# 3DAnimals/3DAnimals

Measured on AMD Instinct MI355X. Metric: train images/sec fwd+bwd @256x256 b16, higher is better.
Workload: dtype f32

## Files before the change

3danimals_amd/_lib.py:

```python
from __future__ import annotations

import ctypes
import os
from typing import NamedTuple

import torch

_HERE = os.path.dirname(os.path.abspath(__file__))
LIB_PATH = os.environ.get("A3D_LIB") or os.path.join(_HERE, "lib", "liba3d_hip.so")

_c_int, _c_float, _c_size_t, _p = ctypes.c_int, ctypes.c_float, ctypes.c_size_t, ctypes.c_void_p


class DmtetOrder(ctypes.Structure):
    _fields_ = [("size", ctypes.c_uint32), ("group_slots", ctypes.c_int32), ("vertex_of_rank", _p), ("edges_ranked", _p), ("edge_of_row", _p),
                ("tets_ranked", _p), ("tet_of_row", _p), ("edge_groups", _p), ("tet_groups", _p)]


class RastOpts(ctypes.Structure):
    _fields_ = [("size", ctypes.c_uint32), ("lists_stride", ctypes.c_int32), ("prev_rast", _p), ("cover_scratch", _p), ("aa_screen", _p),
                ("aa_count", _p), ("topo_off", _p), ("topo_adj", _p), ("topo_opp", _p), ("normals_v_a", _p), ("normals_v_b", _p),
                ("normals_off", _p), ("normals_adj", _p), ("normals_acc_a", _p), ("normals_a", _p), ("normals_acc_b", _p), ("normals_b", _p),
                ("normals_B_a", ctypes.c_int32), ("normals_B_b", ctypes.c_int32), ("defer_resolve", ctypes.c_int32), ("reserved", ctypes.c_int32)]

# ... 253 lines not shown
        "a3d_field_head_scratch_bytes": (_c_size_t, [ctypes.c_int64, _c_int]),
        "a3d_field_head_fwd": (_c_int, [_p, _p, _p, _p, _c_int, ctypes.c_int64, _c_int, _p, _p, _p]),
        "a3d_field_head_bwd": (_c_int, [_p, _p, _p, _p, _p, _c_int, ctypes.c_int64, _c_int, _p, _p, _p, _p]),
    }, {}, {"A3D_FIELD_HEAD_WIDTH": FIELD_HEAD_WIDTH, "A3D_FIELD_HEAD_MAX_C": FIELD_HEAD_MAX_C, "A3D_FIELD_HEAD_WG_ROWS": FIELD_HEAD_WG_ROWS,
            "A3D_FIELD_HEAD_ACT_NONE": FIELD_HEAD_ACT_NONE, "A3D_FIELD_HEAD_ACT_SIGMOID": FIELD_HEAD_ACT_SIGMOID}),
    Surface("a3d_eval.h", {
        "a3d_vertex_visibility_fwd": (_c_int, [_p, _p, _c_int, _c_int, _c_int, _c_int, _c_int, _p, _p, _p]),
        "a3d_nearest_visible_vertex_scratch_bytes": (_c_size_t, [_c_int, _c_int]),
        "a3d_nearest_visible_vertex_slab": (_c_int, [_c_int, _c_int]),
        "a3d_nearest_visible_vertex_fwd": (_c_int, [_p, _p, _p, _c_int, _c_int, _c_int, _p, _p, _p]),
    }, {}, {"A3D_NVV_THREADS": NVV_THREADS, "A3D_NVV_MAX_TRIPS": NVV_MAX_TRIPS, "A3D_NVV_KEYPOINT_TILE": NVV_KEYPOINT_TILE}),
)
SIGNATURES = {name: sig for s in SURFACES for name, sig in s.signatures.items()}
assert len(SIGNATURES) == sum(len(s.signatures) for s in SURFACES), "an entry point is registered in two surfaces"

ABI_VERSION = 405
_lib = None


class A3DError(RuntimeError):
    pass


def lib():
    global _lib
    if _lib is None:
        if not os.path.exists(LIB_PATH):
            raise A3DError(
                f"{LIB_PATH} is missing: build it with `python 3danimals_amd/csrc/build.py` "
                "(or __graft_entry__.build()).  There is no CPU fallback for the HIP hot path."
            )
        handle = ctypes.CDLL(LIB_PATH)
        for name, (res, args) in SIGNATURES.items():
            fn = getattr(handle, name)
            fn.restype, fn.argtypes = res, args
        if handle.a3d_version() != ABI_VERSION:
            raise A3DError(f"{LIB_PATH} has ABI version {handle.a3d_version()}, this package binds version {ABI_VERSION}: rebuild it "
                           "with `python 3danimals_amd/csrc/build.py`")
        _lib = handle
    return _lib


class KernelTimer:

    active = None

    def __init__(self):
        self.records = {}
# ... 22 lines not shown
guard_stats = dict(checks=0, buffers_checked=0, allocations=0)


def set_guard(level):
    global GUARD
    import importlib

    prev, GUARD = GUARD, int(level)
    ops = importlib.import_module(__package__ + ".ops")
    ops.torch = GuardedTorch(torch) if GUARD else torch
    if not GUARD:
        _guard_live.clear()
    return prev


def guarded_empty(shape, dtype, device, zero=False, site=""):
    dtype = dtype or torch.get_default_dtype()
    shape = tuple(int(v) for v in shape)
    n = 1
    for v in shape:
        n *= v
    item = torch.empty((), dtype=dtype).element_size()
    nbytes = n * item
    pad = (-nbytes) % 16
    base = torch.empty(GUARD_BYTES + nbytes + pad + GUARD_BYTES, dtype=torch.uint8, device=device)
    base[:GUARD_BYTES] = _GUARD_BYTE
    base[GUARD_BYTES + nbytes:] = _GUARD_BYTE
    t = base[GUARD_BYTES:GUARD_BYTES + nbytes].view(dtype).view(shape)
    if zero:
        t.zero_()
    elif GUARD >= 2 and n:
        if dtype.is_floating_point:
            t.fill_(float("nan"))
# ... 76 lines not shown
            first = int((t != _GUARD_BYTE).nonzero()[0])
            bad.append(f"{what}: bytes AFTER the buffer overwritten ({int((t != _GUARD_BYTE).sum())}, first {first} bytes past its end)")
            t.fill_(_GUARD_BYTE)
        if not head:
            base[:GUARD_BYTES] = _GUARD_BYTE
    raise A3DError(f"A3D_GUARD: buffer overrun detected after {where}: " + "; ".join(bad))


_HELD = []
_SYNC_EVERY_CALL = os.environ.get("A3D_SYNC_CALLS", "0") == "1"
_TRACE_FILE = open(os.environ["A3D_TRACE_CALLS"], "w") if os.environ.get("A3D_TRACE_CALLS") else None


def call(name: str, *args, tag: str = ""):
    timer = KernelTimer.active
    if _TRACE_FILE is not None:
        _TRACE_FILE.write(f"{name}{tag} {args}\n")
        _TRACE_FILE.flush()
    if timer is not None:
        a, b = torch.cuda.Event(enable_timing=True), torch.cuda.Event(enable_timing=True)
        a.record()
    rc = getattr(lib(), name)(*args)
    del _HELD[:]
    if GUARD and rc == 0:
        guard_check(name + tag)
    if _SYNC_EVERY_CALL:
        try:
            torch.cuda.synchronize()
        except Exception as e:
            raise A3DError(f"{name}{tag}: device fault surfaced after this call: {e}") from e
    if timer is not None:
        b.record()
        timer.records.setdefault(name + tag, []).append((a, b))
    if rc != 0:
        raise A3DError(f"{name} failed ({rc}): {lib().a3d_last_error().decode()}")


def stream() -> int:
    return torch.cuda.current_stream().cuda_stream


# ... 104 lines not shown
```

3danimals_amd/csrc/embed.hip:

```cpp
#include "a3d_common.h"

namespace {

__global__ __launch_bounds__(256) void he_fwd_kernel(const float* __restrict__ x, const float* __restrict__ freq, int n, int symmetrize,
                                                     int ones, long long total, int C, float* __restrict__ out) {
    const long long i = (long long)blockIdx.x * blockDim.x + threadIdx.x;
    if (i >= total) return;
    const int slots = 3 * n + 3 + ones;
    const long long p = i / slots;
    const int q = (int)(i - p * slots);
    float* o = out + p * C;
    if (q < 3 * n) {
        const int c = q / n, k = q - c * n;
        float xv = x[3 * p + c];
        if (symmetrize && c == 0) xv = fabsf(xv);
        float sn, cs;
        sincosf(xv * freq[k], &sn, &cs);
        o[3 + q] = sn;
        o[3 + 3 * n + q] = cs;
    } else if (q < 3 * n + 3) {
        const int j = q - 3 * n;
        const float v = x[3 * p + j];
        o[j] = (symmetrize && j == 0) ? fabsf(v) : v;
    } else {
// ... 11 lines not shown
    const float xv = (symmetrize && c == 0) ? fabsf(raw) : raw;
    const float* gp = g + p * C;
    float acc = gp[c];
    const float* gs = gp + 3 + c * n;
    const float* gc = gs + 3 * n;
    for (int k = 0; k < n; ++k) {
        const float f = freq[k];
        float sn, cs;
        sincosf(xv * f, &sn, &cs);
        acc += f * (gs[k] * cs - gc[k] * sn);
    }
    if (symmetrize && c == 0) acc *= raw > 0.f ? 1.f : (raw < 0.f ? -1.f : 0.f);
    g_x[i] = acc;
}

}

extern "C" int a3d_harmonic_embed_fwd(const float* x, const float* freq, int n, int symmetrize, int ones, int64_t P, float* out,
                                      a3d_stream_t stream) {
    A3D_CHECK_ARG(P >= 0 && n > 0 && (ones == 0 || ones == 1));
    if (P == 0) return A3D_OK;
    A3D_CHECK_ARG(x && freq && out);
    const int C = 3 + 6 * n + ones;
    const long long total = (long long)P * (3 * n + 3 + ones);
    hipLaunchKernelGGL(he_fwd_kernel, dim3(a3d_div_up(total, 256)), dim3(256), 0, (hipStream_t)stream, x, freq, n, symmetrize, ones, total, C, out);
    A3D_LAUNCH_CHECK();
    return A3D_OK;
}

extern "C" int a3d_harmonic_embed_bwd(const float* g_out, const float* x, const float* freq, int n, int symmetrize, int ones, int64_t P,
// ... 10 lines not shown
```

3danimals_amd/csrc/fieldhead.hip:

```cpp
#include "../../include/a3d_fields.h"
#include "a3d_common.h"

namespace {

typedef float f32x4 __attribute__((ext_vector_type(4)));

constexpr int FH_K = A3D_FIELD_HEAD_WIDTH;
constexpr int FH_WAVES = 4;
constexpr int FH_TILE = 16;
constexpr int FH_TILES_PER_WAVE = 8;
constexpr int FH_WAVE_ROWS = FH_TILE * FH_TILES_PER_WAVE;
static_assert(FH_WAVE_ROWS * FH_WAVES == A3D_FIELD_HEAD_WG_ROWS && FH_K == 256, "the header states the work-group's rows");
constexpr int FH_WPAD = FH_K + 16;
constexpr int FH_RED_SEGS = 16;

__device__ __forceinline__ f32x4 fh_load4(const float* p) { return *reinterpret_cast<const f32x4*>(p); }
__device__ __forceinline__ float fh_sigmoid(float x) { return 1.f / (1.f + expf(-x)); }
template <bool ACT>
__device__ __forceinline__ float fh_adjoint(float g, float s, float scale) {
    g = g * scale;
    return ACT ? g * ((1.f - s) * s) : g;
}

__global__ __launch_bounds__(64 * FH_WAVES, 2) void fh_fwd_kernel(const float* __restrict__ h, const float* __restrict__ W,
// ... 169 lines not shown
    for (; w + 8 <= w1; w += 8) {
        float v[8];
#pragma unroll
        for (int u = 0; u < 8; ++u) v[u] = p[(size_t)(w + u) * n];
#pragma unroll
        for (int u = 0; u < 8; ++u) acc += v[u];
    }
    for (; w < w1; ++w) acc += p[(size_t)w * n];
    runs[seg][i] = acc;
    __syncthreads();
    if (seg == 0) {
        float t = runs[0][i];
#pragma unroll
        for (int k = 1; k < FH_RED_SEGS; ++k) t += runs[k][i];
        g_W[e] = t;
    }
}

inline bool fh_sizes_ok(int64_t M, int C) { return M >= 1 && M < (1ll << 31) && C >= 1 && C <= A3D_FIELD_HEAD_MAX_C; }
inline int fh_work_groups(int64_t M) { return (int)((M + A3D_FIELD_HEAD_WG_ROWS - 1) / A3D_FIELD_HEAD_WG_ROWS); }
inline bool fh_aligned16(const void* p) { return ((uintptr_t)p & 15) == 0; }

}

extern "C" size_t a3d_field_head_scratch_bytes(int64_t M, int C) {
    if (!fh_sizes_ok(M, C)) return 0;
    return (size_t)fh_work_groups(M) * C * FH_K * sizeof(float);
}

extern "C" int a3d_field_head_fwd(const float* h, const float* W, const float* lo, const float* scale, int act, int64_t M, int C, float* s,
// ... 20 lines not shown
    const int n_wg = fh_work_groups(M);
    const dim3 grid(n_wg), block(64 * FH_WAVES);
    float* partial = (float*)scratch;
    const bool sig = act == A3D_FIELD_HEAD_ACT_SIGMOID;
    switch ((C + 3) / 4) {
        case 1: fh_launch_bwd<1>(sig, grid, block, st, g_out, s, h, W, scale, (long long)M, C, g_h, partial); break;
        case 2: fh_launch_bwd<2>(sig, grid, block, st, g_out, s, h, W, scale, (long long)M, C, g_h, partial); break;
        case 3: fh_launch_bwd<3>(sig, grid, block, st, g_out, s, h, W, scale, (long long)M, C, g_h, partial); break;
        default: fh_launch_bwd<4>(sig, grid, block, st, g_out, s, h, W, scale, (long long)M, C, g_h, partial); break;
    }
    A3D_LAUNCH_CHECK();
    hipLaunchKernelGGL(fh_reduce_kernel, dim3(C * FH_K / 16), dim3(16 * FH_RED_SEGS), 0, st, partial, n_wg, C * FH_K, g_W);
    A3D_LAUNCH_CHECK();
    return A3D_OK;
}
```

3danimals_amd/csrc/gemm.hip:

```cpp
#include "a3d_common.h"

namespace {

typedef float f32x16 __attribute__((ext_vector_type(16)));
typedef float f32x4 __attribute__((ext_vector_type(4)));

constexpr int GM_N = 256, GM_BK = 32, GM_APAD = GM_BK + 1;

template <int WM, int WN, int BN, int OCC, bool MASK>
__global__ __launch_bounds__(64 * WM * WN, OCC) void gm_nn_kernel(const float* __restrict__ A, const float* __restrict__ B,
                                                                  const float* __restrict__ X, int M, int K, float* __restrict__ C) {
    constexpr int BM = 32 * WM, NT = 64 * WM * WN, TN = BN / WN / 32;
    constexpr int A_F4 = BM * GM_BK / 4 / NT;
    constexpr int B_F4 = GM_BK * BN / 4 / NT;
    static_assert(A_F4 >= 1 && B_F4 >= 1 && BM * GM_BK / 4 % NT == 0 && GM_BK * BN / 4 % NT == 0, "tile / thread count mismatch");
    constexpr int A_ROWS_PER_PASS = NT / 8;
    constexpr int B_ROWS_PER_PASS = NT / (BN / 4);
    __shared__ float As[BM * GM_APAD];
    __shared__ float Bs[GM_BK * BN];
    const int tid = threadIdx.x, lane = tid & 63, wave = tid >> 6, wm = wave / WN, wn = wave - wm * WN;
    const long long m0 = (long long)blockIdx.x * BM;
    const int n0 = blockIdx.y * BN;

    f32x16 acc[TN];
// ... 175 lines not shown
            const long long m = mrow + (r & 3) + 8 * (r >> 2);
            unsigned long long wv = 0ull;
            if (MASK) wv = sign_w[(2 * kh + ((r & 3) >> 1) + 4 * (r >> 2)) * 4 + (row & 3)] >> ((r & 1) * 32 + (row >> 2));
            if (m < M) {
#pragma unroll
                for (int j = 0; j < TN; ++j) {
                    float v = acc[j][r];
                    if (MASK) v = (wv >> (8 * j)) & 1ull ? v : 0.f;
                    C[m * GM_N + n0 + 32 * j + row] = v;
                }
            }
        }
    }
}

inline bool gm_aligned16(const void* p) { return ((uintptr_t)p & 15) == 0; }

}

extern "C" int a3d_gemm_nn_relumask(const float* A, const float* B, const float* X, int64_t M, int N, int K, float* C, a3d_stream_t stream) {
    A3D_CHECK_ARG(M >= 0 && N == GM_N && K > 0 && K % GM_BK == 0 && M < 0x7fffffffll);
    A3D_CHECK_ARG(X == nullptr || K >= 256);
    if (M == 0) return A3D_OK;
    A3D_CHECK_ARG(A && B && C);
    A3D_CHECK_ARG(gm_aligned16(A) && gm_aligned16(B) && gm_aligned16(X));
    hipStream_t s = (hipStream_t)stream;
    if (K == 256) {
        static int n_cu_of[64] = {0};
        int dev = 0;
        A3D_HIP(hipGetDevice(&dev));
        A3D_CHECK_ARG(dev >= 0 && dev < 64);
        if (!n_cu_of[dev]) {
// ... 20 lines not shown
```

3danimals_amd/hostnets.py:

```python
from __future__ import annotations

import torch
import torch.nn as nn
import torch.nn.functional as F


REFERENCE_FORMULATION = False


def reference_formulation(enable=True):
    global REFERENCE_FORMULATION
    REFERENCE_FORMULATION = bool(enable)
    return REFERENCE_FORMULATION


def _activation(name):
    table = {"tanh": nn.Tanh, "sigmoid": nn.Sigmoid, "relu": nn.ReLU}
    if name not in table:
        raise NotImplementedError(name)
    return table[name]()


class HarmonicEmbedding(nn.Module):

# ... 142 lines not shown
        return out

    @staticmethod
    @torch.autograd.function.once_differentiable
    def backward(ctx, g):
        from . import ops

        saved = ctx.saved_tensors
        x_emb, w_in, index, w_first, w_head, scale, s = saved[:7]
        hidden, ys = saved[7:7 + ctx.n_hidden], saved[7 + ctx.n_hidden:]
        g, g_head = ops.field_head_bwd(g, s, ys[-1], w_head, scale, ctx.act)
        g_x, g_in, g_rows, g_first, g_hidden = _stack_backward(g, x_emb, w_in, index, w_first, hidden, ys, ctx.n_images, ctx.needs_input_grad[0])
        return (g_x, g_in, g_rows, None, g_first, g_head, None, None, None, *g_hidden)


def _long_list(x, weight):
    return (x.is_cuda and x.dim() == 2 and x.shape[0] >= SPLITK_MIN_ROWS and x.shape[0] % SPLITK_PARTS == 0 and x.is_contiguous()
            and x.dtype == torch.float32 and torch.is_grad_enabled() and weight.requires_grad)


def linear(x, weight, bias=None):
    if bias is None and _long_list(x, weight):
        return _LinearSplitK.apply(x, weight)
    return F.linear(x, weight, bias)


def linear_relu(x, weight, bias=None):
    if _long_list(x, weight):
        return _LinearReLUSplitK.apply(x, weight, bias)
    if (x.is_cuda and x.dim() == 2 and x.shape[0] >= SPLITK_MIN_ROWS and x.dtype == torch.float32
# ... 73 lines not shown
    @property
    def indexed_feat(self):
        return not REFERENCE_FORMULATION

    def forward(self, x, feat=None, feat_index=None):
        assert (feat is None and self.extra_feat_dim == 0) or (feat.shape[-1] == self.extra_feat_dim)
        if REFERENCE_FORMULATION:
            return self._forward_reference(x, feat if feat_index is None or feat is None else feat[feat_index])
        if feat_index is not None and feat is not None and x.dim() == 2 and isinstance(self.mlp.network[0], nn.Linear) \
                and self.mlp.network[0].bias is None:
            return self._forward_indexed(x, feat, feat_index)
        if feat_index is not None and feat is not None:
            feat = feat[feat_index]
        if feat is None and self._stack_ok(x, False):
            return self._stacked(x, None, None)
        if feat is None and self._fused_input_ok(x):
            out = self.mlp(self._fused_input(x))
            if self.min_max is not None:
                out = out * (self.min_max[:, 1] - self.min_max[:, 0]) + self.min_max[:, 0]
            return out
        if self.symmetrize:
            x = torch.cat([x[..., :1].abs(), x[..., 1:]], -1)
        h = x
        if self.embedder is not None:
            h = self.embedder(x)
            if self.embed_concat_pts:
                h = torch.cat([x, h], -1)
        if feat is None:
            out = self.mlp(linear_relu(h, self.in_layer.weight, self.in_layer.bias))
        else:
# ... 27 lines not shown
        out = self.mlp(self.relu(x_in))
        if self.min_max is not None:
            out = out * (self.min_max[:, 1] - self.min_max[:, 0]) + self.min_max[:, 0]
        return out

    def _fused_input_ok(self, x):
        return (x.is_cuda and x.dim() == 2 and x.shape[1] == 3 and x.shape[0] >= SPLITK_MIN_ROWS and x.dtype == torch.float32
                and self.embedder is not None and self.embed_concat_pts and self.in_layer.bias is not None)

    def _fused_input(self, x):
        from . import ops

        h = ops.harmonic_embed(x, self.embedder._frequencies(x.device), symmetrize=self.symmetrize, ones=True)
        weight = torch.cat([self.in_layer.weight, self.in_layer.bias[:, None]], dim=1)
        return linear_relu(h, weight, None)

    def _stack_ok(self, x, with_feat):
        if not (USE_FIELD_STACK and self._fused_input_ok(x) and torch.is_grad_enabled() and x.shape[0] % SPLITK_PARTS == 0
                and self.in_layer.weight.requires_grad and self.in_layer.weight.shape[0] == 256):
            return False
        layers = list(self.mlp.network)
        n_pairs = 0
        while 2 * n_pairs + 1 < len(layers) and isinstance(layers[2 * n_pairs], nn.Linear) and isinstance(layers[2 * n_pairs + 1], nn.ReLU):
            lin = layers[2 * n_pairs]
            want_in = 256 + (self.extra_feat_dim if (with_feat and n_pairs == 0) else 0)
            if lin.bias is not None or tuple(lin.weight.shape) != (256, want_in):
                return False
            n_pairs += 1
        return n_pairs >= 1

# ... 153 lines not shown
```

3danimals_amd/ops.py:

```python
from __future__ import annotations

import ctypes
import math
import os
import struct
from collections import OrderedDict

import torch

from . import _lib
from ._lib import call, f32c, f32h, ptr, require_device, stream


class _IdentityCache:

    def __init__(self, maxsize=8):
        self.maxsize = maxsize
        self.data = OrderedDict()

    @staticmethod
    def key(t):
        return (t.data_ptr(), tuple(t.shape), t.dtype, t._version)

    def get(self, t, make):
# ... 1916 lines not shown
        out = torch.empty((P, 3 + 6 * n + int(ones)), dtype=torch.float32, device=x.device)
        call("a3d_harmonic_embed_fwd", ptr(x), ptr(freq), n, int(symmetrize), int(ones), P, ptr(out), stream())
        ctx.save_for_backward(x, freq)
        ctx.cfg = (int(symmetrize), int(ones))
        return out

    @staticmethod
    @torch.autograd.function.once_differentiable
    def backward(ctx, g):
        x, freq = ctx.saved_tensors
        g_x = torch.empty_like(x)
        call("a3d_harmonic_embed_bwd", ptr(f32h(g)), ptr(x), ptr(freq), freq.shape[0], ctx.cfg[0], ctx.cfg[1], x.shape[0], ptr(g_x), stream())
        return g_x, None, None, None


def harmonic_embed(x, freq, symmetrize=False, ones=False):
    if x.dim() != 2 or x.shape[1] != 3 or freq.dim() != 1 or freq.shape[0] < 1:
        raise ValueError(f"harmonic_embed: expected x [P,3] and n >= 1 frequencies [n], got {list(x.shape)} and {list(freq.shape)}")
    if not (x.is_floating_point() and freq.is_floating_point()):
        raise ValueError(f"harmonic_embed: x and freq must be floating point, got {x.dtype} and {freq.dtype}")
    return _HarmonicEmbed.apply(x, freq, bool(symmetrize), bool(ones))


def gemm_nn_relumask(a, b, x=None):
    if a.dim() != 2 or b.dim() != 2 or a.shape[1] < 32 or a.shape[1] % 32 or tuple(b.shape) != (a.shape[1], 256):
        raise ValueError(f"gemm_nn_relumask: expected a [M,K] and b [K,256] with K a positive multiple of 32, got {list(a.shape)} and {list(b.shape)}")
    if x is not None and (tuple(x.shape) != (a.shape[0], 256) or x.dtype != torch.float32 or not x.is_contiguous() or a.shape[1] < 256):
        raise ValueError(f"gemm_nn_relumask: the mask must be float32, contiguous and [M,256] = [{a.shape[0]},256], with K >= 256; got {x.dtype} "
                         f"{list(x.shape)} with strides {list(x.stride())} and K = {a.shape[1]}")
    require_device(a, b, x, what="gemm_nn_relumask")
    a, b = f32c(a), f32c(b)
    M, K = a.shape
    c = torch.empty((M, 256), dtype=torch.float32, device=a.device)
    call("a3d_gemm_nn_relumask", ptr(a), ptr(b), ptr(x), M, 256, K, ptr(c), stream())
    return c


def _field_head_args(what, h, weight, scale, act):
    if h.dim() != 2 or weight.dim() != 2 or h.shape[1] != _lib.FIELD_HEAD_WIDTH or weight.shape[1] != _lib.FIELD_HEAD_WIDTH \
            or not 1 <= weight.shape[0] <= _lib.FIELD_HEAD_MAX_C or not 1 <= h.shape[0] < 1 << 31:
        raise ValueError(f"{what}: expected h [M,{_lib.FIELD_HEAD_WIDTH}] with M >= 1 and weight [C <= {_lib.FIELD_HEAD_MAX_C},{_lib.FIELD_HEAD_WIDTH}], "
                         f"got {list(h.shape)} and {list(weight.shape)}")
    if act not in (_lib.FIELD_HEAD_ACT_NONE, _lib.FIELD_HEAD_ACT_SIGMOID):
        raise ValueError(f"{what}: act is 0 (none) or 1 (sigmoid), got {act!r}")
    if scale is not None and tuple(scale.shape) != (weight.shape[0],):
        raise ValueError(f"{what}: scale / lo must be [C] = [{weight.shape[0]}], got {list(scale.shape)}")
    return int(h.shape[0]), int(weight.shape[0])


def field_head_fwd(h, weight, lo=None, scale=None, act=0):
# ... 1099 lines not shown
```

Baseline: 1071.

## Add fused HIP path for SDF field gradient with custom JVP and split-K GEMMs

Adds a dedicated path for fields that need the gradient of their output with respect to input points. It uses a harmonic-embedding JVP kernel, masked NT GEMMs, a field-grad head kernel and a split-K TN GEMM for weight gradients, replacing generic autograd double-backward. The path runs only when the field matches a strict structural check. Instrumentation and guarded allocations are also skipped during CUDA graph capture. This adds a large amount of custom kernel code and a narrow eligibility check, so some models may silently fall back to the old path.

```diff
diff --git a/3danimals_amd/_lib.py b/3danimals_amd/_lib.py
--- a/3danimals_amd/_lib.py
+++ b/3danimals_amd/_lib.py
@@ -291,6 +291,17 @@
 SIGNATURES = {name: sig for s in SURFACES for name, sig in s.signatures.items()}
 assert len(SIGNATURES) == sum(len(s.signatures) for s in SURFACES), "an entry point is registered in two surfaces"
 
+FIELD_GRAD_SIGNATURES = {
+    "a3d_gemm_nt_relumask": (_c_int, [_p, _p, _p, ctypes.c_int64, _c_int, _c_int, _p, _p]),
+    "a3d_harmonic_embed_jvp": (_c_int, [_p, _p, _p, _c_int, _c_int, _c_int, ctypes.c_int64, _p, _p]),
+    "a3d_field_grad_head_fwd": (_c_int, [_p, _p, _p, ctypes.c_int64, _p, _p]),
+    "a3d_field_grad_head_scratch_bytes": (_c_size_t, [ctypes.c_int64]),
+    "a3d_field_grad_head_bwd": (_c_int, [_p, _p, _p, ctypes.c_int64, _p, _p, _p, _p]),
+    "a3d_gemm_tn_splitk_scratch_bytes": (_c_size_t, [ctypes.c_int64, _c_int, _c_int]),
+    "a3d_gemm_tn_splitk": (_c_int, [_p, _p, ctypes.c_int64, _c_int, _c_int, _p, _p, _p]),
+}
+assert not set(FIELD_GRAD_SIGNATURES) & set(SIGNATURES)
+
 ABI_VERSION = 405
 _lib = None
 
@@ -308,7 +319,7 @@
                 "(or __graft_entry__.build()).  There is no CPU fallback for the HIP hot path."
             )
         handle = ctypes.CDLL(LIB_PATH)
-        for name, (res, args) in SIGNATURES.items():
+        for name, (res, args) in list(SIGNATURES.items()) + list(FIELD_GRAD_SIGNATURES.items()):
             fn = getattr(handle, name)
             fn.restype, fn.argtypes = res, args
         if handle.a3d_version() != ABI_VERSION:
@@ -361,9 +372,15 @@
     return prev
 
 
+def _capturing():
+    return torch.cuda.is_available() and torch.cuda.is_current_stream_capturing()
+
+
 def guarded_empty(shape, dtype, device, zero=False, site=""):
     dtype = dtype or torch.get_default_dtype()
     shape = tuple(int(v) for v in shape)
+    if _capturing():
+        return torch.zeros(shape, dtype=dtype, device=device) if zero else torch.empty(shape, dtype=dtype, device=device)
     n = 1
     for v in shape:
         n *= v
@@ -470,6 +487,9 @@
 
 def call(name: str, *args, tag: str = ""):
     timer = KernelTimer.active
+    aids = (GUARD or _SYNC_EVERY_CALL or timer is not None) and not _capturing()
+    if not aids:
+        timer = None
     if _TRACE_FILE is not None:
         _TRACE_FILE.write(f"{name}{tag} {args}\n")
         _TRACE_FILE.flush()
@@ -478,9 +498,9 @@
         a.record()
     rc = getattr(lib(), name)(*args)
     del _HELD[:]
-    if GUARD and rc == 0:
+    if GUARD and rc == 0 and aids:
         guard_check(name + tag)
-    if _SYNC_EVERY_CALL:
+    if _SYNC_EVERY_CALL and aids:
         try:
             torch.cuda.synchronize()
         except Exception as e:
diff --git a/3danimals_amd/csrc/embed.hip b/3danimals_amd/csrc/embed.hip
--- a/3danimals_amd/csrc/embed.hip
+++ b/3danimals_amd/csrc/embed.hip
@@ -1,4 +1,5 @@
 #include "a3d_common.h"
+#include "fieldgrad.h"
 
 namespace {
 
@@ -49,6 +50,45 @@
     g_x[i] = acc;
 }
 
+__global__ __launch_bounds__(256) void he_jvp_kernel(const float* __restrict__ x, const float* __restrict__ lam, const float* __restrict__ freq,
+                                                     int n, int symmetrize, int ones, long long total, int C, float* __restrict__ out) {
+    const long long i = (long long)blockIdx.x * blockDim.x + threadIdx.x;
+    if (i >= total) return;
+    const int slots = 3 * n + 3 + ones;
+    const long long p = i / slots;
+    const int q = (int)(i - p * slots);
+    float* o = out + p * C;
+    if (q == 3 * n + 3) {
+        o[C - 1] = 0.f;
+        return;
+    }
+    const int c = q < 3 * n ? q / n : q - 3 * n;
+    const float raw = x[3 * p + c];
+    float l = lam[3 * p + c];
+    if (symmetrize && c == 0) l *= raw > 0.f ? 1.f : (raw < 0.f ? -1.f : 0.f);
+    if (q < 3 * n) {
+        const float f = freq[q - c * n];
+        float sn, cs;
+        sincosf(((symmetrize && c == 0) ? fabsf(raw) : raw) * f, &sn, &cs);
+        o[3 + q] = l * (f * cs);
+        o[3 + 3 * n + q] = -(l * (f * sn));
+    } else {
+        o[c] = l;
+    }
+}
+
+}
+
+extern "C" int a3d_harmonic_embed_jvp(const float* x, const float* lam, const float* freq, int n, int symmetrize, int ones, int64_t P,
+                                      float* d_emb, a3d_stream_t stream) {
+    A3D_CHECK_ARG(P >= 0 && n > 0 && (ones == 0 || ones == 1));
+    if (P == 0) return A3D_OK;
+    A3D_CHECK_ARG(x && lam && freq && d_emb);
+    const long long total = (long long)P * (3 * n + 3 + ones);
+    hipLaunchKernelGGL(he_jvp_kernel, dim3(a3d_div_up(total, 256)), dim3(256), 0, (hipStream_t)stream, x, lam, freq, n, symmetrize, ones, total,
+                       3 + 6 * n + ones, d_emb);
+    A3D_LAUNCH_CHECK();
+    return A3D_OK;
 }
 
 extern "C" int a3d_harmonic_embed_fwd(const float* x, const float* freq, int n, int symmetrize, int ones, int64_t P, float* out,
diff --git a/3danimals_amd/csrc/fieldgrad.h b/3danimals_amd/csrc/fieldgrad.h
--- /dev/null
+++ b/3danimals_amd/csrc/fieldgrad.h
@@ -0,0 +1,30 @@
+#ifndef A3D_FIELDGRAD_H
+#define A3D_FIELDGRAD_H
+
+#include "../../include/a3d.h"
+
+#ifdef __cplusplus
+extern "C" {
+#endif
+
+
+int a3d_gemm_nt_relumask(const float* A, const float* B, const float* X, int64_t M, int N, int K, float* C, a3d_stream_t stream);
+
+int a3d_harmonic_embed_jvp(const float* x, const float* lam, const float* freq, int n, int symmetrize, int ones, int64_t P, float* d_emb,
+                           a3d_stream_t stream);
+
+int a3d_field_grad_head_fwd(const float* s, const float* w, const float* y, int64_t M, float* b, a3d_stream_t stream);
+
+size_t a3d_field_grad_head_scratch_bytes(int64_t M);
+
+int a3d_field_grad_head_bwd(const float* s, const float* t, const float* w, int64_t M, void* scratch, float* g_w, float* g_s,
+                            a3d_stream_t stream);
+
+size_t a3d_gemm_tn_splitk_scratch_bytes(int64_t M, int NQ, int batch);
+
+int a3d_gemm_tn_splitk(const float* P, const float* Q, int64_t M, int NQ, int batch, void* scratch, float* C, a3d_stream_t stream);
+
+#ifdef __cplusplus
+}
+#endif
+#endif
diff --git a/3danimals_amd/csrc/fieldhead.hip b/3danimals_amd/csrc/fieldhead.hip
--- a/3danimals_amd/csrc/fieldhead.hip
+++ b/3danimals_amd/csrc/fieldhead.hip
@@ -1,4 +1,5 @@
 #include "../../include/a3d_fields.h"
+#include "fieldgrad.h"
 #include "a3d_common.h"
 
 namespace {
@@ -207,6 +208,41 @@
 #pragma unroll
         for (int k = 1; k < FH_RED_SEGS; ++k) t += runs[k][i];
         g_W[e] = t;
+    }
+}
+
+__global__ __launch_bounds__(256) void fg_head_fwd_kernel(const float* __restrict__ s, const float* __restrict__ w, const float* __restrict__ y,
+                                                          long long M, float* __restrict__ b) {
+    const long long i = (long long)blockIdx.x * blockDim.x + threadIdx.x;
+    if (i >= M * (FH_K / 4)) return;
+    const long long m = i / (FH_K / 4);
+    const int k4 = (int)(i - m * (FH_K / 4));
+    const float sv = s[m];
+    const f32x4 wv = fh_load4(w + 4 * k4), yv = fh_load4(y + 4 * i);
+    f32x4 d;
+#pragma unroll
+    for (int r = 0; r < 4; ++r) d[r] = yv[r] > 0.f ? sv * wv[r] : 0.f;
+    *reinterpret_cast<f32x4*>(b + 4 * i) = d;
+}
+
+constexpr int FG_ROWS = 64;
+
+__global__ __launch_bounds__(FH_K) void fg_head_bwd_kernel(const float* __restrict__ s, const float* __restrict__ t, const float* __restrict__ w,
+                                                           long long M, float* __restrict__ partial, float* __restrict__ g_s) {
+    const int k = threadIdx.x;
+    const long long m0 = (long long)blockIdx.x * FG_ROWS;
+    const int rows = (int)(M - m0 < FG_ROWS ? M - m0 : FG_ROWS);
+    float acc = 0.f;
+    for (int r = 0; r < rows; ++r) acc += s[m0 + r] * t[(m0 + r) * FH_K + k];
+    partial[(size_t)blockIdx.x * FH_K + k] = acc;
+    if (g_s != nullptr) {
+        const int lane = k & 63, wave = k >> 6;
+        const f32x4 wv = fh_load4(w + 4 * lane);
+        for (int r = wave; r < rows; r += FH_K / 64) {
+            const f32x4 tv = fh_load4(t + (m0 + r) * FH_K + 4 * lane);
+            const float v = a3d_wave_sum((tv[0] * wv[0] + tv[1] * wv[1]) + (tv[2] * wv[2] + tv[3] * wv[3]));
+            if (lane == 0) g_s[m0 + r] = v;
+        }
     }
 }
 
@@ -257,3 +293,29 @@
     A3D_LAUNCH_CHECK();
     return A3D_OK;
 }
+
+extern "C" size_t a3d_field_grad_head_scratch_bytes(int64_t M) {
+    if (M < 1 || M >= (1ll << 31)) return 0;
+    return (size_t)((M + FG_ROWS - 1) / FG_ROWS) * FH_K * sizeof(float);
+}
+
+extern "C" int a3d_field_grad_head_fwd(const float* s, const float* w, const float* y, int64_t M, float* b, a3d_stream_t stream) {
+    A3D_CHECK_ARG(M >= 1 && M < (1ll << 31));
+    A3D_CHECK_ARG(s && w && y && b && fh_aligned16(w) && fh_aligned16(y) && fh_aligned16(b));
+    hipLaunchKernelGGL(fg_head_fwd_kernel, dim3(a3d_div_up(M * (FH_K / 4), 256)), dim3(256), 0, (hipStream_t)stream, s, w, y, (long long)M, b);
+    A3D_LAUNCH_CHECK();
+    return A3D_OK;
+}
+
+extern "C" int a3d_field_grad_head_bwd(const float* s, const float* t, const float* w, int64_t M, void* scratch, float* g_w, float* g_s,
+                                       a3d_stream_t stream) {
+    A3D_CHECK_ARG(M >= 1 && M < (1ll << 31));
+    A3D_CHECK_ARG(s && t && w && scratch && g_w && fh_aligned16(t) && fh_aligned16(w));
+    const int n_wg = (int)((M + FG_ROWS - 1) / FG_ROWS);
+    hipStream_t st = (hipStream_t)stream;
+    hipLaunchKernelGGL(fg_head_bwd_kernel, dim3(n_wg), dim3(FH_K), 0, st, s, t, w, (long long)M, (float*)scratch, g_s);
+    A3D_LAUNCH_CHECK();
+    hipLaunchKernelGGL(fh_reduce_kernel, dim3(FH_K / 16), dim3(16 * FH_RED_SEGS), 0, st, (const float*)scratch, n_wg, FH_K, g_w);
+    A3D_LAUNCH_CHECK();
+    return A3D_OK;
+}
diff --git a/3danimals_amd/csrc/gemm.hip b/3danimals_amd/csrc/gemm.hip
--- a/3danimals_amd/csrc/gemm.hip
+++ b/3danimals_amd/csrc/gemm.hip
@@ -1,4 +1,5 @@
 #include "a3d_common.h"
+#include "fieldgrad.h"
 
 namespace {
 
@@ -213,8 +214,204 @@
     }
 }
 
+constexpr int GS_BM = 64, GS_BN = 128, GS_NT = 256;
+
+template <bool MASK>
+__global__ __launch_bounds__(GS_NT, 2) void gm_short_kernel(const float* __restrict__ A, const float* __restrict__ B,
+                                                            const float* __restrict__ X, int M, int K, float* __restrict__ C) {
+    constexpr int BNP = GS_BN + 1, TN = 2;
+    __shared__ float As[GS_BM * GM_APAD];
+    __shared__ float Bs[GM_BK * BNP];
+    const int tid = threadIdx.x, lane = tid & 63, wave = tid >> 6, wm = wave >> 1, wn = wave & 1;
+    const int m0 = blockIdx.x * GS_BM;
+    const int n0 = blockIdx.y * GS_BN;
+    f32x16 acc[TN];
+#pragma unroll
+    for (int j = 0; j < TN; ++j)
+#pragma unroll
+        for (int r = 0; r < 16; ++r) acc[j][r] = 0.f;
+    const f32x4 zero4 = {0.f, 0.f, 0.f, 0.f};
+    const int a_row = tid >> 3, a_kq = tid & 7;
+    const float* a_src = A + (long long)(m0 + a_row) * K + 4 * a_kq;
+    const int b_row = tid >> 3, b_q = tid & 7;
+    const float* b_src = B + (long long)(n0 + b_row) * K + 4 * b_q;
+    f32x4 ra[2], rb[4];
+    auto load_chunk = [&](int k0) {
+#pragma unroll
+        for (int i = 0; i < 2; ++i)
+            ra[i] = (m0 + a_row + 32 * i < M && k0 + 4 * a_kq < K) ? *reinterpret_cast<const f32x4*>(a_src + (long long)32 * i * K + k0) : zero4;
+#pragma unroll
+        for (int i = 0; i < 4; ++i) rb[i] = k0 + 4 * b_q < K ? *reinterpret_cast<const f32x4*>(b_src + (long long)32 * i * K + k0) : zero4;
+    };
+    load_chunk(0);
+    for (int k0 = 0; k0 < K; k0 += GM_BK) {
+        __syncthreads();
+#pragma unroll
+        for (int i = 0; i < 2; ++i) {
+            float* d = As + (a_row + 32 * i) * GM_APAD + 4 * a_kq;
+            d[0] = ra[i].x; d[1] = ra[i].y; d[2] = ra[i].z; d[3] = ra[i].w;
+        }
+#pragma unroll
+        for (int i = 0; i < 4; ++i) {
+            float* d = Bs + (4 * b_q) * BNP + b_row + 32 * i;
+            d[0] = rb[i].x; d[BNP] = rb[i].y; d[2 * BNP] = rb[i].z; d[3 * BNP] = rb[i].w;
+        }
+        __syncthreads();
+        if (k0 + GM_BK < K) load_chunk(k0 + GM_BK);
+        const float* a_base = As + (32 * wm + (lane & 31)) * GM_APAD + (lane >> 5);
+        const float* b_base = Bs + (lane >> 5) * BNP + 64 * wn + (lane & 31);
+#pragma unroll
+        for (int kk = 0; kk < GM_BK; kk += 2) {
+            const float av = a_base[kk];
+#pragma unroll
+            for (int j = 0; j < TN; ++j) acc[j] = __builtin_amdgcn_mfma_f32_32x32x2f32(av, b_base[kk * BNP + 32 * j], acc[j], 0, 0, 0);
+        }
+    }
+    const int col0 = n0 + 64 * wn + (lane & 31);
+#pragma unroll
+    for (int r = 0; r < 16; ++r) {
+        const int m = m0 + 32 * wm + 4 * (lane >> 5) + (r & 3) + 8 * (r >> 2);
+        if (m < M) {
+#pragma unroll
+            for (int j = 0; j < TN; ++j) {
+                const long long at = (long long)m * GM_N + col0 + 32 * j;
+                float v = acc[j][r];
+                if (MASK) v = X[at] > 0.f ? v : 0.f;
+                C[at] = v;
+            }
+        }
+    }
+}
+
+constexpr int GT_T = 128, GT_NT = 256;
+
+__global__ __launch_bounds__(GT_NT, 2) void gm_tn_kernel(const float* __restrict__ P, const float* __restrict__ Q, int M, int NQ, int batch,
+                                                         int splits, int rows_per_split, float* __restrict__ out) {
+    __shared__ __attribute__((aligned(16))) float Ps[GM_BK * GT_T];
+    __shared__ __attribute__((aligned(16))) float Qs[GM_BK * GT_T];
+    const int tid = threadIdx.x, lane = tid & 63, wave = tid >> 6, wm = wave >> 1, wn = wave & 1;
+    const int n0 = blockIdx.x * GT_T, c0 = blockIdx.y * GT_T, b = blockIdx.z / splits, sp = blockIdx.z - b * splits;
+    const int m_begin = sp * rows_per_split, m_end = min(M, m_begin + rows_per_split);
+    P += (long long)b * M * GM_N;
+    Q += (long long)b * M * NQ;
+    f32x16 acc[2][2];
+#pragma unroll
+    for (int i = 0; i < 2; ++i)
+#pragma unroll
+        for (int j = 0; j < 2; ++j)
+#pragma unroll
+            for (int r = 0; r < 16; ++r) acc[i][j][r] = 0.f;
+    const f32x4 zero4 = {0.f, 0.f, 0.f, 0.f};
+    const int l_row = tid >> 5, l_c4 = tid & 31;
+    const bool q_col = n0 + 4 * l_c4 < NQ;
+    f32x4 rp[4], rq[4];
+    auto load_chunk = [&](int m0) {
+#pragma unroll
+        for (int i = 0; i < 4; ++i) {
+            const int m = m0 + l_row + 8 * i;
+            rp[i] = m < m_end ? *reinterpret_cast<const f32x4*>(P + (long long)m * GM_N + c0 + 4 * l_c4) : zero4;
+            rq[i] = m < m_end && q_col ? *reinterpret_cast<const f32x4*>(Q + (long long)m * NQ + n0 + 4 * l_c4) : zero4;
+        }
+    };
+    load_chunk(m_begin);
+    for (int m0 = m_begin; m0 < m_end; m0 += GM_BK) {
+        __syncthreads();
+#pragma unroll
+        for (int i = 0; i < 4; ++i) {
+            *reinterpret_cast<f32x4*>(Ps + (l_row + 8 * i) * GT_T + 4 * l_c4) = rp[i];
+            *reinterpret_cast<f32x4*>(Qs + (l_row + 8 * i) * GT_T + 4 * l_c4) = rq[i];
+        }
+        __syncthreads();
+        if (m0 + GM_BK < m_end) load_chunk(m0 + GM_BK);
+        const float* p_base = Ps + (lane >> 5) * GT_T + 64 * wm + (lane & 31);
+        const float* q_base = Qs + (lane >> 5) * GT_T + 64 * wn + (lane & 31);
+#pragma unroll
+        for (int kk = 0; kk < GM_BK; kk += 2) {
+            const float a0 = p_base[kk * GT_T], a1 = p_base[kk * GT_T + 32], b0 = q_base[kk * GT_T], b1 = q_base[kk * GT_T + 32];
+            acc[0][0] = __builtin_amdgcn_mfma_f32_32x32x2f32(a0, b0, acc[0][0], 0, 0, 0);
+            acc[0][1] = __builtin_amdgcn_mfma_f32_32x32x2f32(a0, b1, acc[0][1], 0, 0, 0);
+            acc[1][0] = __builtin_amdgcn_mfma_f32_32x32x2f32(a1, b0, acc[1][0], 0, 0, 0);
+            acc[1][1] = __builtin_amdgcn_mfma_f32_32x32x2f32(a1, b1, acc[1][1], 0, 0, 0);
+        }
+    }
+    float* dst = out + ((long long)sp * batch + b) * GM_N * NQ;
+#pragma unroll
+    for (int i = 0; i < 2; ++i)
+#pragma unroll
+        for (int j = 0; j < 2; ++j) {
+            const int col = n0 + 64 * wn + 32 * j + (lane & 31);
+            if (col < NQ) {
+#pragma unroll
+                for (int r = 0; r < 16; ++r) {
+                    const int row = c0 + 64 * wm + 32 * i + (r & 3) + 8 * (r >> 2) + 4 * (lane >> 5);
+                    dst[(long long)row * NQ + col] = acc[i][j][r];
+                }
+            }
+        }
+}
+
+__global__ __launch_bounds__(256) void gm_tn_reduce_kernel(const float* __restrict__ partial, int splits, long long n4, float* __restrict__ C) {
+    const long long i = (long long)blockIdx.x * blockDim.x + threadIdx.x;
+    if (i >= n4) return;
+    f32x4 v = *reinterpret_cast<const f32x4*>(partial + 4 * i);
+    int s = 1;
+    for (; s + 8 <= splits; s += 8) {
+        f32x4 t[8];
+#pragma unroll
+        for (int u = 0; u < 8; ++u) t[u] = *reinterpret_cast<const f32x4*>(partial + 4 * ((long long)(s + u) * n4 + i));
+#pragma unroll
+        for (int u = 0; u < 8; ++u) v += t[u];
+    }
+    for (; s < splits; ++s) v += *reinterpret_cast<const f32x4*>(partial + 4 * ((long long)s * n4 + i));
+    *reinterpret_cast<f32x4*>(C + 4 * i) = v;
+}
+
+inline int gm_tn_splits(int64_t M, int NQ, int batch) {
+    const long long tiles = (long long)a3d_div_up(NQ, GT_T) * (GM_N / GT_T) * batch;
+    long long want = (512 + tiles - 1) / tiles;
+    const long long most = a3d_div_up(M, GM_BK);
+    want = want > 32 ? 32 : want;
+    return (int)(want < 1 ? 1 : (want > most ? most : want));
+}
+inline bool gm_tn_sizes_ok(int64_t M, int NQ, int batch) {
+    return M >= 1 && M < 0x7fffff00ll && NQ >= 4 && NQ <= GM_N && NQ % 4 == 0 && batch >= 1 && batch <= 64;
+}
+
 inline bool gm_aligned16(const void* p) { return ((uintptr_t)p & 15) == 0; }
 
+}
+
+extern "C" size_t a3d_gemm_tn_splitk_scratch_bytes(int64_t M, int NQ, int batch) {
+    if (!gm_tn_sizes_ok(M, NQ, batch)) return 0;
+    return (size_t)gm_tn_splits(M, NQ, batch) * batch * GM_N * NQ * sizeof(float);
+}
+
+extern "C" int a3d_gemm_tn_splitk(const float* P, const float* Q, int64_t M, int NQ, int batch, void* scratch, float* C, a3d_stream_t stream) {
+    A3D_CHECK_ARG(gm_tn_sizes_ok(M, NQ, batch));
+    A3D_CHECK_ARG(P && Q && C && scratch);
+    A3D_CHECK_ARG(gm_aligned16(P) && gm_aligned16(Q) && gm_aligned16(C) && gm_aligned16(scratch));
+    const int splits = gm_tn_splits(M, NQ, batch);
+    const int rows_per_split = a3d_div_up(a3d_div_up(M, splits), GM_BK) * GM_BK;
+    hipStream_t s = (hipStream_t)stream;
+    const dim3 grid(a3d_div_up(NQ, GT_T), GM_N / GT_T, batch * splits);
+    hipLaunchKernelGGL(gm_tn_kernel, grid, dim3(GT_NT), 0, s, P, Q, (int)M, NQ, batch, splits, rows_per_split, (float*)scratch);
+    A3D_LAUNCH_CHECK();
+    const long long n4 = (long long)batch * GM_N * NQ / 4;
+    hipLaunchKernelGGL(gm_tn_reduce_kernel, dim3(a3d_div_up(n4, 256)), dim3(256), 0, s, (const float*)scratch, splits, n4, C);
+    A3D_LAUNCH_CHECK();
+    return A3D_OK;
+}
+
+extern "C" int a3d_gemm_nt_relumask(const float* A, const float* B, const float* X, int64_t M, int N, int K, float* C, a3d_stream_t stream) {
+    A3D_CHECK_ARG(M >= 0 && N == GM_N && K > 0 && K % 4 == 0 && M < 0x7fffff00ll);
+    if (M == 0) return A3D_OK;
+    A3D_CHECK_ARG(A && B && C);
+    A3D_CHECK_ARG(gm_aligned16(A) && gm_aligned16(B));
+    const dim3 grid(a3d_div_up(M, GS_BM), GM_N / GS_BN), block(GS_NT);
+    if (X) hipLaunchKernelGGL((gm_short_kernel<true>), grid, block, 0, (hipStream_t)stream, A, B, X, (int)M, K, C);
+    else hipLaunchKernelGGL((gm_short_kernel<false>), grid, block, 0, (hipStream_t)stream, A, B, X, (int)M, K, C);
+    A3D_LAUNCH_CHECK();
+    return A3D_OK;
 }
 
 extern "C" int a3d_gemm_nn_relumask(const float* A, const float* B, const float* X, int64_t M, int N, int K, float* C, a3d_stream_t stream) {
diff --git a/3danimals_amd/hostnets.py b/3danimals_amd/hostnets.py
--- a/3danimals_amd/hostnets.py
+++ b/3danimals_amd/hostnets.py
@@ -180,6 +180,115 @@
         return (g_x, g_in, g_rows, None, g_first, g_head, None, None, None, *g_hidden)
 
 
+USE_FIELD_GRAD = True
+
+
+def _tn_products(p, q):
+    from . import ops
+
+    return ops.gemm_tn_splitk(p, q)
+
+
+def _field_grad_chain(s, y, w_head, hidden):
+    from . import ops
+
+    n_hidden = len(hidden)
+    b = torch.empty_like(y)
+    ops.field_grad_head_fwd(s, w_head, y[n_hidden], out=b[n_hidden])
+    for l in range(n_hidden, 0, -1):
+        ops.gemm_nn_relumask(b[l], hidden[l - 1], y[l - 1], out=b[l - 1])
+    return b
+
+
+class _FieldInputGrad(torch.autograd.Function):
+
+    @staticmethod
+    def forward(ctx, s, x, y, w_in, w_head, freq, symmetrize, *hidden):
+        from . import ops
+
+        b = _field_grad_chain(s, y, w_head, hidden)
+        ctx.save_for_backward(s, x, y, w_in, w_head, freq, b, *hidden)
+        ctx.symmetrize = symmetrize
+        return ops.harmonic_embed_bwd_raw(b[0].mm(w_in), x, freq, symmetrize, True)
+
+    @staticmethod
+    @torch.autograd.function.once_differentiable
+    def backward(ctx, lam):
+        from . import ops
+
+        s, x, y, w_in, w_head, freq, b = ctx.saved_tensors[:7]
+        hidden = ctx.saved_tensors[7:]
+        n_hidden = len(hidden)
+        need = ctx.needs_input_grad
+        dv = ops.harmonic_embed_jvp(x, lam, freq, ctx.symmetrize, True)
+        t = torch.empty_like(y)
+        ops.gemm_nt_relumask(dv, w_in, y[0], out=t[0])
+        for l in range(1, n_hidden + 1):
+            ops.gemm_nt_relumask(t[l - 1], hidden[l - 1], y[l], out=t[l])
+        g_in = _tn_products(b[:1], dv[None])[0] if need[3] else None
+        g_head, g_s = ops.field_grad_head_bwd(s, t[n_hidden], w_head, need_s=need[0]) if (need[4] or need[0]) else (None, None)
+        g_hidden = [None] * n_hidden
+        if any(need[7:]):
+            prods = _tn_products(b[1:], t[:-1])
+            g_hidden = [prods[l] if need[7 + l] else None for l in range(n_hidden)]
+        return (g_s, None, None, g_in, g_head if need[4] else None, None, None, *g_hidden)
+
+
+class _FieldWeightTap(torch.autograd.Function):
+
+    @staticmethod
+    def forward(ctx, box, m, w_in, w_head, *hidden):
+        ctx.box = box
+        ctx.save_for_backward(w_head, *hidden)
+        return torch.empty((m, 1), dtype=w_in.dtype, device=w_in.device)
+
+    @staticmethod
+    @torch.autograd.function.once_differentiable
+    def backward(ctx, s):
+        e, y = ctx.box["e"], ctx.box["y"]
+        w_head, hidden = ctx.saved_tensors[0], ctx.saved_tensors[1:]
+        need = ctx.needs_input_grad
+        b = _field_grad_chain(s, y, w_head, hidden)
+        g_in = _tn_products(b[:1], e[None])[0] if need[2] else None
+        g_head = s.reshape(1, -1).mm(y[-1]) if need[3] else None
+        g_hidden = [None] * len(hidden)
+        if any(need[4:]):
+            prods = _tn_products(b[1:], y[:-1])
+            g_hidden = [prods[l] if need[4 + l] else None for l in range(len(hidden))]
+        return (None, None, g_in, g_head, *g_hidden)
+
+
+class _FieldValue(torch.autograd.Function):
+
+    @staticmethod
+    def forward(ctx, x, tap, box, w_in, w_head, freq, symmetrize, *hidden):
+        from . import ops
+
+        e = ops.harmonic_embed_raw(x, freq, symmetrize, True)
+        y = torch.empty((len(hidden) + 1, x.shape[0], 256), dtype=torch.float32, device=x.device)
+        zero = _zero_bias(e, w_in)
+        torch._addmm_activation(zero, e, w_in.t(), use_gelu=False, out=y[0])
+        for l, w in enumerate(hidden):
+            torch._addmm_activation(zero, y[l], w.t(), use_gelu=False, out=y[l + 1])
+        box.update(e=e, y=y)
+        ctx.save_for_backward(x, y, w_in, w_head, freq, *hidden)
+        ctx.symmetrize = bool(symmetrize)
+        return y[-1].mm(w_head.t())
+
+    @staticmethod
+    def backward(ctx, s):
+        x, y, w_in, w_head, freq = ctx.saved_tensors[:5]
+        hidden = ctx.saved_tensors[5:]
+        g_x = _FieldInputGrad.apply(s, x.detach(), y, w_in, w_head, freq, ctx.symmetrize, *hidden) if ctx.needs_input_grad[0] else None
+        return (g_x, s if ctx.needs_input_grad[1] else None, None, None, None, None, None, *([None] * len(hidden)))
+
+
+def _field_value(x, w_in, w_head, freq, symmetrize, *hidden):
+    box = {}
+    tap = _FieldWeightTap.apply(box, x.shape[0], w_in, w_head, *hidden)
+    return _FieldValue.apply(x, tap, box, w_in, w_head, freq, symmetrize, *hidden)
+
+
 def _long_list(x, weight):
     return (x.is_cuda and x.dim() == 2 and x.shape[0] >= SPLITK_MIN_ROWS and x.shape[0] % SPLITK_PARTS == 0 and x.is_contiguous()
             and x.dtype == torch.float32 and torch.is_grad_enabled() and weight.requires_grad)
@@ -283,6 +392,8 @@
             feat = feat[feat_index]
         if feat is None and self._stack_ok(x, False):
             return self._stacked(x, None, None)
+        if feat is None and self._field_grad_ok(x):
+            return self._field_grad(x)
         if feat is None and self._fused_input_ok(x):
             out = self.mlp(self._fused_input(x))
             if self.min_max is not None:
@@ -340,6 +451,29 @@
         h = ops.harmonic_embed(x, self.embedder._frequencies(x.device), symmetrize=self.symmetrize, ones=True)
         weight = torch.cat([self.in_layer.weight, self.in_layer.bias[:, None]], dim=1)
         return linear_relu(h, weight, None)
+
+    def _field_grad_ok(self, x):
+        if not (USE_FIELD_GRAD and x.is_cuda and x.dtype == torch.float32 and x.dim() == 2 and x.shape[1] == 3 and 1 <= x.shape[0] < SPLITK_MIN_ROWS
+                and x.requires_grad and torch.is_grad_enabled() and self.embedder is not None and self.embed_concat_pts
+                and len(self.embedder.frequencies) % 2 == 0 and self.in_layer.bias is not None and self.in_layer.weight.shape[0] == 256
+                and self.in_layer.weight.dtype == torch.float32 and self.min_max is None and self.extra_feat_dim == 0):
+            return False
+        layers = list(self.mlp.network)
+        if len(layers) < 3 or len(layers) % 2 == 0:
+            return False
+        for i, layer in enumerate(layers[:-1]):
+            if i % 2 == 1 and not isinstance(layer, nn.ReLU):
+                return False
+            if i % 2 == 0 and not (isinstance(layer, nn.Linear) and layer.bias is None and tuple(layer.weight.shape) == (256, 256)):
+                return False
+        head = layers[-1]
+        return isinstance(head, nn.Linear) and head.bias is None and tuple(head.weight.shape) == (1, 256) and head.weight.dtype == torch.float32
+
+    def _field_grad(self, x):
+        w_in = torch.cat([self.in_layer.weight, self.in_layer.bias[:, None]], dim=1)
+        layers = list(self.mlp.network)
+        return _field_value(x, w_in, layers[-1].weight, self.embedder._frequencies(x.device), bool(self.symmetrize),
+                            *[l.weight for l in layers[:-1:2]])
 
     def _stack_ok(self, x, with_feat):
         if not (USE_FIELD_STACK and self._fused_input_ok(x) and torch.is_grad_enabled() and x.shape[0] % SPLITK_PARTS == 0
diff --git a/3danimals_amd/ops.py b/3danimals_amd/ops.py
--- a/3danimals_amd/ops.py
+++ b/3danimals_amd/ops.py
@@ -1954,6 +1954,26 @@
         return g_x, None, None, None
 
 
+def harmonic_embed_raw(x, freq, symmetrize, ones):
+    return _HarmonicEmbed.forward(_NoCtx(), x, freq, symmetrize, ones)
+
+
+def harmonic_embed_bwd_raw(g, x, freq, symmetrize, ones):
+    require_device(g, x, freq, what="harmonic_embed_bwd")
+    x, freq = f32c(x), f32c(freq)
+    if tuple(g.shape) != (x.shape[0], 3 + 6 * freq.shape[0] + int(ones)):
+        raise ValueError(f"harmonic_embed_bwd: g must be [{x.shape[0]},{3 + 6 * freq.shape[0] + int(ones)}], got {list(g.shape)}")
+    g_x = torch.empty_like(x)
+    call("a3d_harmonic_embed_bwd", ptr(f32h(g)), ptr(x), ptr(freq), freq.shape[0], int(symmetrize), int(ones), x.shape[0], ptr(g_x), stream())
+    return g_x
+
+
+class _NoCtx:
+
+    def save_for_backward(self, *tensors):
+        pass
+
+
 def harmonic_embed(x, freq, symmetrize=False, ones=False):
     if x.dim() != 2 or x.shape[1] != 3 or freq.dim() != 1 or freq.shape[0] < 1:
         raise ValueError(f"harmonic_embed: expected x [P,3] and n >= 1 frequencies [n], got {list(x.shape)} and {list(freq.shape)}")
@@ -1962,7 +1982,15 @@
     return _HarmonicEmbed.apply(x, freq, bool(symmetrize), bool(ones))
 
 
-def gemm_nn_relumask(a, b, x=None):
+def _rows256_out(what, out, m, device):
+    if out is None:
+        return torch.empty((m, 256), dtype=torch.float32, device=device)
+    if tuple(out.shape) != (m, 256) or out.dtype != torch.float32 or not out.is_contiguous() or out.device != device:
+        raise ValueError(f"{what}: out must be float32, contiguous and [{m},256] on {device}, got {out.dtype} {list(out.shape)} on {out.device}")
+    return out
+
+
+def gemm_nn_relumask(a, b, x=None, out=None):
     if a.dim() != 2 or b.dim() != 2 or a.shape[1] < 32 or a.shape[1] % 32 or tuple(b.shape) != (a.shape[1], 256):
         raise ValueError(f"gemm_nn_relumask: expected a [M,K] and b [K,256] with K a positive multiple of 32, got {list(a.shape)} and {list(b.shape)}")
     if x is not None and (tuple(x.shape) != (a.shape[0], 256) or x.dtype != torch.float32 or not x.is_contiguous() or a.shape[1] < 256):
@@ -1971,9 +1999,76 @@
     require_device(a, b, x, what="gemm_nn_relumask")
     a, b = f32c(a), f32c(b)
     M, K = a.shape
-    c = torch.empty((M, 256), dtype=torch.float32, device=a.device)
+    c = _rows256_out("gemm_nn_relumask", out, M, a.device)
     call("a3d_gemm_nn_relumask", ptr(a), ptr(b), ptr(x), M, 256, K, ptr(c), stream())
     return c
+
+
+def gemm_nt_relumask(a, w, x=None, out=None):
+    if a.dim() != 2 or w.dim() != 2 or a.shape[1] < 4 or a.shape[1] % 4 or tuple(w.shape) != (256, a.shape[1]):
+        raise ValueError(f"gemm_nt_relumask: expected a [M,K] and w [256,K] with K a positive multiple of 4, got {list(a.shape)} and {list(w.shape)}")
+    if x is not None and (tuple(x.shape) != (a.shape[0], 256) or x.dtype != torch.float32 or not x.is_contiguous()):
+        raise ValueError(f"gemm_nt_relumask: the mask must be float32, contiguous and [M,256] = [{a.shape[0]},256]; got {x.dtype} {list(x.shape)} "
+                         f"with strides {list(x.stride())}")
+    require_device(a, w, x, what="gemm_nt_relumask")
+    a, w = f32c(a), f32c(w)
+    M, K = a.shape
+    c = _rows256_out("gemm_nt_relumask", out, M, a.device)
+    call("a3d_gemm_nt_relumask", ptr(a), ptr(w), ptr(x), M, 256, K, ptr(c), stream(), tag=f"[K{K}]")
+    return c
+
+
+def gemm_tn_splitk(p, q):
+    if p.dim() != 3 or q.dim() != 3 or p.shape[2] != 256 or tuple(q.shape[:2]) != tuple(p.shape[:2]) or not 4 <= q.shape[2] <= 256 or q.shape[2] % 4 \
+            or not 1 <= p.shape[0] <= 64 or p.shape[1] < 1:
+        raise ValueError(f"gemm_tn_splitk: expected p [B,M,256] and q [B,M,C] with 1 <= B <= 64, M >= 1 and C a multiple of 4 up to 256, got "
+                         f"{list(p.shape)} and {list(q.shape)}")
+    require_device(p, q, what="gemm_tn_splitk")
+    p, q = f32c(p), f32c(q)
+    B, M, C = q.shape
+    scratch = torch.empty(_lib.lib().a3d_gemm_tn_splitk_scratch_bytes(M, C, B), dtype=torch.uint8, device=p.device)
+    out = torch.empty((B, 256, C), dtype=torch.float32, device=p.device)
+    call("a3d_gemm_tn_splitk", ptr(p), ptr(q), M, C, B, ptr(scratch), ptr(out), stream(), tag=f"[n{B}x{C}]")
+    return out
+
+
+def harmonic_embed_jvp(x, lam, freq, symmetrize=False, ones=False):
+    if x.dim() != 2 or x.shape[1] != 3 or tuple(lam.shape) != tuple(x.shape) or freq.dim() != 1 or freq.shape[0] < 1:
+        raise ValueError(f"harmonic_embed_jvp: expected x and lam [P,3] and n >= 1 frequencies [n], got {list(x.shape)}, {list(lam.shape)} and "
+                         f"{list(freq.shape)}")
+    require_device(x, lam, freq, what="harmonic_embed_jvp")
+    x, lam, freq = f32c(x), f32c(lam), f32c(freq)
+    P, n = x.shape[0], freq.shape[0]
+    out = torch.empty((P, 3 + 6 * n + int(ones)), dtype=torch.float32, device=x.device)
+    call("a3d_harmonic_embed_jvp", ptr(x), ptr(lam), ptr(freq), n, int(symmetrize), int(ones), P, ptr(out), stream())
+    return out
+
+
+def _field_grad_head_args(what, s, w, y):
+    if y.dim() != 2 or y.shape[1] != _lib.FIELD_HEAD_WIDTH or y.shape[0] < 1 or s.numel() != y.shape[0] or w.numel() != _lib.FIELD_HEAD_WIDTH:
+        raise ValueError(f"{what}: expected s [M] or [M,1], w [256] or [1,256] and [M,256] hidden vectors with M >= 1, got {list(s.shape)}, "
+                         f"{list(w.shape)} and {list(y.shape)}")
+    return int(y.shape[0])
+
+
+def field_grad_head_fwd(s, w, y, out=None):
+    M = _field_grad_head_args("field_grad_head_fwd", s, w, y)
+    require_device(s, w, y, what="field_grad_head_fwd")
+    s, w, y = f32c(s), f32c(w), f32c(y)
+    b = _rows256_out("field_grad_head_fwd", out, M, y.device)
+    call("a3d_field_grad_head_fwd", ptr(s), ptr(w), ptr(y), M, ptr(b), stream())
+    return b
+
+
+def field_grad_head_bwd(s, t, w, need_s=False):
+    M = _field_grad_head_args("field_grad_head_bwd", s, w, t)
+    require_device(s, t, w, what="field_grad_head_bwd")
+    s, t, w = f32c(s), f32c(t), f32c(w)
+    scratch = torch.empty(_lib.lib().a3d_field_grad_head_scratch_bytes(M), dtype=torch.uint8, device=t.device)
+    g_w = torch.empty((1, _lib.FIELD_HEAD_WIDTH), dtype=torch.float32, device=t.device)
+    g_s = torch.empty((M, 1), dtype=torch.float32, device=t.device) if need_s else None
+    call("a3d_field_grad_head_bwd", ptr(s), ptr(t), ptr(w), M, ptr(scratch), ptr(g_w), ptr(g_s), stream())
+    return g_w, g_s
 
 
 def _field_head_args(what, h, weight, scale, act):
```

New measurement: 1092, median of 6. +2.0%, better.
